# zhangxinsong-nlp/XFM

Measured on AMD Instinct MI355X. Metric: image-text pairs/sec fwd+bwd, XFM-base 224px/30tok, higher is better.
Workload: dtype bf16; 1 GPU; Pretrain.py full multimodal step (ITC+ITM+MLM+MIM), XFM-base, synthetic 224px images + 30-token captions, random init; units_per_gpu=64, global_batch=64, dropout=True, ordered_reductions=True, grad_allreduce=False, parallelism=dp1, image_res=224

## Files before the change

### xfm_amd/csrc/gemm.hip

```cpp
#include "gemm_common.h"
#include <limits.h>
#include "gemm_nt_small.hip"
#include "gemm_nt_256.hip"
#include "nt320_gemm.hip"
#include "gemm_tn_small.hip"
#include "gemm_tn_256.hip"
#include "gemm_cast.hip"

static int nt_k_slices(int M, int N, int K) {
  const long t = (long)cdiv(M, 64) * cdiv(N, 128);
  if (K < 8192 || t >= 192) return 1;
  int sp = (int)(512 / t);
  if (sp > K / 1024) sp = K / 1024;
  return sp < 1 ? 1 : sp;
}

static int nt_plan(int M, int N, int K, long lda, long ldb, int epi, int tile_hint, int* rows_a_out, int* k_splits_out) {
  *rows_a_out = 0;
  *k_splits_out = 1;
  if (tile_hint == 6) {
    static const int nt320_env = xfm_env_int("XFM_GEMM_NT320", 1);
    if (nt320_env && nt320_eligible(M, lda, N, ldb, K)) return 6;
    tile_hint = 0;
  }
  int cfg = tile_hint;
  if (cfg <= 0) {
    static const int split_env = xfm_env_int("XFM_GEMM_TAIL_SPLIT", 35);
    const long tn256 = cdiv(N, 256), t256 = (long)cdiv(M, 256) * tn256;
    if (split_env && tile_hint == 0 && M >= 2048 && t256 > 256 && t256 % 256 != 0 && (t256 % 256) * 100 < split_env * 256) {
      const int rows_a = (int)((t256 / 256) * 256 / tn256) * 256;
      if (rows_a > 0 && rows_a < M) {
        if (!nt256_eligible(rows_a, lda, N, ldb)) return 1;
        *rows_a_out = rows_a;
        return 5;
      }
    }
    if (M >= 2048 && (t256 >= 180 || (t256 >= 120 && M >= 8192))) cfg = nt256_eligible(M, lda, N, ldb) ? 5 : 1;
    else if (M >= 2048 && t256 >= 120) cfg = 1;
    else if ((long)cdiv(M, 256) * cdiv(N, 128) >= 768) cfg = 4;
    else if ((long)cdiv(M, 128) * cdiv(N, 128) >= 800) cfg = 1;
    else if ((long)cdiv(M, 64) * cdiv(N, 128) >= 512) cfg = 2;
    else if (K >= 1536 && epi != EPI_F32_ACC && (long)cdiv(M, 64) * cdiv(N, 128) < 300) {
      cfg = 8;
    }
    else if ((long)cdiv(M, 64) * cdiv(N, 128) >= 128 || K >= 1536) {
      cfg = 7;
      if (epi == EPI_F32_ACC) *k_splits_out = nt_k_slices(M, N, K);
    }
    else cfg = 3;
  }
  return cfg;
}

int xfm_gemm_nt_plan_impl(int M, int N, int K, int epi, int tile_hint, int* cfg, int* rows_a) {
  XFM_REQUIRE(M > 0 && N > 0 && K > 0 && cfg != nullptr && rows_a != nullptr, "gemm_nt_plan: bad arguments");
  int ks = 1;
  *cfg = nt_plan(M, N, K, K, K, epi, tile_hint, rows_a, &ks);
  return XFM_OK;
}

static GemmNT gemm_nt_args(const void* A, long lda, const void* B, long ldb, void* C, long ldc, const float* bias, int M, int N, int K) {
  static const int gm_env = xfm_env_int("XFM_GEMM_GROUP_M", 0);
  GemmNT g{};
  g.A = (const bf16*)A; g.lda = lda;
  g.B = (const bf16*)B; g.ldb = ldb;
  g.C = C; g.ldc = ldc;
  g.bias = bias;
  g.M = M; g.N = N; g.K = K;
  g.group_m = gm_env > 0 ? gm_env : 8;
  g.k_splits = 1;
  return g;
}

int xfm_gemm_nt_impl(const void* A, long lda, const void* B, long ldb, void* C, long ldc, const float* bias,
                     void* aux, long ldaux, int M, int N, int K, int epi, int tile_hint, hipStream_t st) {
  XFM_REQUIRE(M > 0 && N > 0 && K > 0, "gemm_nt: empty problem M=%d N=%d K=%d", M, N, K);
  XFM_REQUIRE(K % 64 == 0, "gemm_nt: K=%d must be a multiple of 64", K);
  XFM_REQUIRE(lda % 8 == 0 && ldb % 8 == 0, "gemm_nt: lda=%ld ldb=%ld must be multiples of 8", lda, ldb);
  XFM_REQUIRE(((uintptr_t)A % 16) == 0 && ((uintptr_t)B % 16) == 0 && ((uintptr_t)C % 16) == 0,
              "gemm_nt: operands must be 16-byte aligned");
  XFM_REQUIRE((epi != EPI_GELU && epi != EPI_DGELU) || aux != nullptr, "gemm_nt: epilogue %d needs aux", epi);
  GemmNT g = gemm_nt_args(A, lda, B, ldb, C, ldc, bias, M, N, K);
  g.aux = (bf16*)aux; g.ldaux = ldaux;
  int rows_a = 0, k_splits = 1;
  const int cfg = nt_plan(M, N, K, lda, ldb, epi, tile_hint, &rows_a, &k_splits);
  if (rows_a > 0) {
    int rc = xfm_gemm_nt_impl(A, lda, B, ldb, C, ldc, bias, aux, ldaux, rows_a, N, K, epi, 5, st);
    if (rc != XFM_OK) return rc;
    const long esz = (epi == EPI_F32 || epi == EPI_F32_ACC) ? 4 : 2;
    return xfm_gemm_nt_impl((const bf16*)A + (long)rows_a * lda, lda, B, ldb, (char*)C + (long)rows_a * ldc * esz, ldc, bias,
                            aux ? (void*)((bf16*)aux + (long)rows_a * ldaux) : nullptr, ldaux, M - rows_a, N, K, epi, -1, st);
  }
  g.k_splits = k_splits;
  switch (cfg) {
    case 1: return launch_nt<128, 128, 2>(g, epi, st);
    case 2: return launch_nt<64, 128, 2>(g, epi, st);
    case 7: return launch_nt<64, 128, 3>(g, epi, st);
    case 8: return launch_nt<64, 64, 4>(g, epi, st);
    case 4: return launch_nt_ring(g, epi, st);
    case 5: return launch_nt_256(g, epi, st);
    case 6: return launch_nt_320(g, epi, st);
    default: return launch_nt<64, 64, 2>(g, epi, st);
  }
}

// ... 343 lines not shown
```

### xfm_amd/csrc/nt320_gemm.hip

```cpp

constexpr int NT320_UNIT = 64 * 128;
constexpr int NT320_LEAD = 11;
constexpr int NT320_LDS = 18 * NT320_UNIT;

template <int V>
struct Nt320Phase { static constexpr int v = V; };

__device__ __forceinline__ void nt320_wait(int n) {
  if (n >= 10) wait_vm<10>();
  else if (n == 9) wait_vm<9>();
  else if (n == 8) wait_vm<8>();
  else if (n == 7) wait_vm<7>();
  else if (n == 6) wait_vm<6>();
  else if (n == 5) wait_vm<5>();
  else if (n == 4) wait_vm<4>();
  else if (n == 3) wait_vm<3>();
  else if (n == 2) wait_vm<2>();
  else if (n == 1) wait_vm<1>();
  else wait_vm<0>();
}

template <int EPI>
__global__ __launch_bounds__(512) void gemm_nt_320_kernel(GemmNT g) {
  constexpr int BM = 320, BN = 256, MT = 10, NT = 4, UNIT = NT320_UNIT, LEAD = NT320_LEAD;
  extern __shared__ __attribute__((aligned(16))) char smem[];
  const int tid = threadIdx.x, lane = tid & 63, w = __builtin_amdgcn_readfirstlane(tid >> 6);
  const int wr = w >> 2, wc = w & 3;
  const int lr = lane & 15, lg = lane >> 4;
  const int tiles_n = (g.N + BN - 1) / BN, tiles_m = (g.M + BM - 1) / BM;
  const int nk = g.K / 64;
  int tm, tn;
  grouped_tile(xcd_remap(blockIdx.x, tiles_m * tiles_n), tiles_m, tiles_n, g.group_m, tm, tn);
  const int m0 = tm * BM, n0 = tn * BN;

  unsigned soff[9];
  {
    const int ur = w * 8 + (lane >> 3);
#pragma unroll
    for (int u = 0; u < 5; ++u) {
      const int r = (ur & 31) + 32 * u + (ur >> 5) * 160;
      int gr = m0 + r; gr = gr < g.M ? gr : g.M - 1;
      soff[u == 0 ? 0 : 4 + u] = (unsigned)gr * (unsigned)g.lda + (((lane & 7) ^ swz_x(r)) << 3);
    }
#pragma unroll
    for (int h = 0; h < 4; ++h) {
      const int r = h * 64 + ur;
      int gr = n0 + r; gr = gr < g.N ? gr : g.N - 1;
      soff[1 + h] = (unsigned)gr * (unsigned)g.ldb + (((lane & 7) ^ swz_w(r)) << 3);
    }
  }
  const unsigned lds0 = (unsigned)(uintptr_t)LDS_PTR(void, smem) + (unsigned)(w * 1024);
  auto issue = [&](int j, int kt) {
    if (kt >= nk) return;
    const bf16* src = ((j == 0 || j >= 5) ? g.A : g.B) + kt * 64;
    const unsigned lds_addr = lds0 + (unsigned)(((kt & 1) * 9 + j) * UNIT);
    asm volatile("s_mov_b32 m0, %1\n\ts_nop 0\n\tglobal_load_lds_dwordx4 %0, off" ::"v"(src + (size_t)soff[j]), "s"(lds_addr) : "memory", "m0");
  };

  f32x4 acc[MT][NT];
#pragma unroll
  for (int i = 0; i < MT; ++i)
#pragma unroll
    for (int j = 0; j < NT; ++j) acc[i][j] = f32x4{0.f, 0.f, 0.f, 0.f};

  const int xs = swz_x(lr);
  const int wu = 8 * (lr >> 2) + (lr & 3);
  const int ws = swz_w(wu);
  const int xbase0 = (wr * 32 + lr) * 128 + (((0 + lg) ^ xs) << 4), xbase1 = (wr * 32 + lr) * 128 + (((4 + lg) ^ xs) << 4);
  const int wbase0 = (1 + wc) * UNIT + wu * 128 + (((0 + lg) ^ ws) << 4), wbase1 = (1 + wc) * UNIT + wu * 128 + (((4 + lg) ^ ws) << 4);

  bf16x8 xa[2][2], wf[4][2];
  const int total = 9 * nk;

  auto phase = [&](auto P, int kt) {
    constexpr int p = decltype(P)::v;
    constexpr int cum = p == 4 ? 9 : 2 * (p + 1);
    constexpr int need = p == 4 ? 14 : 6 + p;
    if (p == 0) { issue(2, kt + 1); issue(3, kt + 1); }
    if (p == 1) { issue(4, kt + 1); issue(5, kt + 1); }
    if (p == 2) { issue(6, kt + 1); issue(7, kt + 1); }
    if (p == 3) { issue(8, kt + 1); issue(0, kt + 2); }
    if (p == 4) { issue(1, kt + 2); }
    const char* buf = smem + (kt & 1) * 9 * UNIT;
    const char* xslot = buf + (p == 0 ? 0 : 4 + p) * UNIT;
#pragma unroll
    for (int m = 0; m < 2; ++m) {
      xa[m][0] = *reinterpret_cast<const bf16x8*>(xslot + xbase0 + m * 2048);
      xa[m][1] = *reinterpret_cast<const bf16x8*>(xslot + xbase1 + m * 2048);
    }
    if (p == 0) {
#pragma unroll
      for (int n = 0; n < 4; ++n) {
        wf[n][0] = *reinterpret_cast<const bf16x8*>(buf + wbase0 + (n >> 1) * 4096 + (n & 1) * 512);
        wf[n][1] = *reinterpret_cast<const bf16x8*>(buf + wbase1 + (n >> 1) * 4096 + (n & 1) * 512);
      }
    }
    {
      const int rem = total - 9 * kt;
      if (rem >= LEAD + cum) wait_vm<LEAD + cum - need>();
      else nt320_wait(rem - need);
    }
    XFM_BAR();
    __builtin_amdgcn_s_setprio(1);
#pragma unroll
    for (int ks = 0; ks < 2; ++ks)
#pragma unroll
      for (int m = 0; m < 2; ++m)
#pragma unroll
        for (int n = 0; n < 4; ++n)
          acc[2 * p + m][n] = __builtin_amdgcn_mfma_f32_16x16x32_bf16(wf[n][ks], xa[m][ks], acc[2 * p + m][n], 0, 0, 0);
    __builtin_amdgcn_s_setprio(0);
    XFM_BAR();
  };

#pragma unroll
  for (int j = 0; j < 9; ++j) issue(j, 0);
  issue(0, 1);
  issue(1, 1);
  nt320_wait((LEAD < total ? LEAD : total) - 5);
  XFM_BAR();
  if (wr == 1) XFM_BAR();

  for (int kt = 0; kt < nk; ++kt) {
    phase(Nt320Phase<0>{}, kt);
    phase(Nt320Phase<1>{}, kt);
    phase(Nt320Phase<2>{}, kt);
    phase(Nt320Phase<3>{}, kt);
    phase(Nt320Phase<4>{}, kt);
  }
  if (wr == 0) XFM_BAR();
  if (EPI == EPI_DGELU) {
    gemm_epilogue<MT / 2, NT, EPI>(g, reinterpret_cast<f32x4(&)[MT / 2][NT]>(acc[0]), m0 + wr * 160, n0 + wc * 64, lr, lg);
    gemm_epilogue<MT / 2, NT, EPI>(g, reinterpret_cast<f32x4(&)[MT / 2][NT]>(acc[MT / 2]), m0 + wr * 160 + 80, n0 + wc * 64, lr, lg);
  } else {
    gemm_epilogue<MT, NT, EPI>(g, acc, m0 + wr * 160, n0 + wc * 64, lr, lg);
  }
}

static bool nt320_eligible(int M, long lda, int N, long ldb, int K) {
  static const int cus = xfm_cu_count() > 0 ? xfm_cu_count() : 256;
  return N % 256 == 0 && K % 64 == 0 && (long)cdiv(M, 320) * (N / 256) <= cus && nt256_eligible(M, lda, N, ldb);
}

static int launch_nt_320(const GemmNT& g, int epi, hipStream_t st) {
  if (!nt320_eligible(g.M, g.lda, g.N, g.ldb, g.K)) {
    xfm_set_error("gemm_nt: M=%d N=%d K=%d is no shape of the one-round 320x256 kernel", g.M, g.N, g.K);
    return XFM_E_ARG;
  }
  const int tiles = cdiv(g.M, 320) * (g.N / 256);
  const int rc = nt_with_epilogue(epi, [&](auto e) {
    constexpr int E = decltype(e)::value;
    lds_launch<gemm_nt_320_kernel<E>, NT320_LDS>(dim3(tiles), dim3(512), NT320_LDS, st, g);
  });
  return rc != XFM_OK ? rc : xfm_check_launch("gemm_nt_320");
}
```

### xfm_amd/side_stream.py

```python
import contextlib
import os

import torch

from . import functional as Fx
from . import marks as _marks


class _DeferredCall:
    persistent = False

    def __init__(self, fn, keep=()):
        self.fn, self.keep = fn, tuple(keep)

    def run(self):
        self.fn()


class _WgradStream:
    _streams = {}
    enabled = os.environ.get("XFM_WGRAD_STREAM", "1") != "0"
    priority = int(os.environ.get("XFM_WGRAD_PRIO", "0"))

    @classmethod
    def side_of(cls, device, launch):
        key = (device.index if device.index is not None else torch.cuda.current_device(), launch.cuda_stream)
        if key not in cls._streams:
            cls._streams[key] = torch.cuda.Stream(device=device, priority=cls.priority)
        return cls._streams[key]

    @classmethod
    def sides(cls, device_index):
        return {launch: side for (d, launch), side in list(cls._streams.items()) if d == device_index}

    def __init__(self, device, label=None):
        self.label = label
        if label is not None:
            _marks.mark(label + " begin")
        self.main = torch.cuda.current_stream(device)
        if label is not None:
            from .arena import grads_ready
            grads_ready(device)
        self.on = _WgradStream.enabled
        if self.on:
            self.side = _WgradStream.side_of(device, self.main)
            self.side.wait_stream(self.main)
        self.keep = []
        self.queue = []
        self.reduces = []

    def _hand_over(self, keep):
        if not self.on:
            return contextlib.nullcontext()
        ev = torch.cuda.Event()
        ev.record(self.main)
        self.side.wait_event(ev)
        self.keep.append(keep)
        return torch.cuda.stream(self.side)

    def defer_tn(self, dy, x, dw, dbias=None):
        self.queue.append((dy, x, dw, dbias))

    def defer_call(self, fn, keep=()):
        self.reduces.append(_DeferredCall(fn, keep))

    def defer_reduces(self, rq):
        self.reduces.append(rq)

    def flush(self):
        reduces = self.reduces
        self.reduces = [r for r in reduces if getattr(r, "persistent", False)]
        items, self.queue = self.queue, []
        if not (reduces or items):
            return
        by_m = {}
        for it in items:
            by_m.setdefault(it[0].shape[0], []).append(it)
        with self._hand_over((items, reduces)):
            for r in reduces:
                r.run()
            for group in by_m.values():
                Fx.gemm_tn_group(group)

    def gemm_tn(self, dy, x, dw, **kw):
        with self._hand_over((dy, x)):
            Fx.gemm_tn(dy, x, dw, **kw)

    def project(self, x, slot):
        if not self.on:
            return Fx.gemm_nt(x, slot.wb, slot.b), None
        with torch.cuda.stream(self.side):
            y = Fx.gemm_nt(x, slot.wb, slot.b)
            ev = torch.cuda.Event()
            ev.record(self.side)
        y.record_stream(self.main)
        return y, ev

    def take(self, pair):
        y, ev = pair
        if ev is not None:
            self.main.wait_event(ev)
        return y

    def run(self, fn, keep=()):
        with self._hand_over(tuple(keep)):
            return fn()

    def sync_side(self):
        if self.on:
            self.main.wait_stream(self.side)

    def join_at_end(self):
        self.flush()
        if self.on:
            main, side, keep = self.main, self.side, self.keep

            def rejoin():
                main.wait_stream(side)
                cur = torch.cuda.current_stream(main.device)
                if cur != main:
                    cur.wait_stream(side)
                keep.clear()
            torch.autograd.Variable._execution_engine.queue_callback(rejoin)
            self.keep = []
        else:
            self.keep.clear()

    def join(self):
        if self.label is not None:
            _marks.mark(self.label + " chain end")
        self.flush()
        if self.on:
            self.main.wait_stream(self.side)
        self.keep.clear()
        if self.label is not None:
            _marks.mark(self.label + " end")
```

### xfm_amd/vit_trunk.py

```python
import math
import os

import torch
import torch.nn as nn

from . import _lib
from . import functional as Fx
from .arena import LinearSlot, OwnsArena, ParamArena, arena_note_grad, arena_note_use, grad_of
from .ops import linear_slot
from .side_stream import _WgradStream

_FAST_DELTA = os.environ.get("XFM_ATTN_FAST_DELTA", "0") != "0"
_VIT_FUSED_BWD = os.environ.get("XFM_ATTN_VIT_BWD", "0") != "0"
_DEFER_WGRAD = os.environ.get("XFM_VIT_DEFER_WGRAD", "1") != "0"
_RELPOS_AHEAD = os.environ.get("XFM_VIT_RELPOS_AHEAD", "1") != "0"
_DEFER_LN = os.environ.get("XFM_VIT_DEFER_LN", "1") != "0"
_WGRAD_GROUP_BLOCKS = int(os.environ.get("XFM_VIT_WGRAD_GROUP", "0"))
_GRAD_CHUNK_BLOCKS = max(1, int(os.environ.get("XFM_VIT_GRAD_CHUNK", "4")))


class _Affine(nn.Module):

    def __init__(self, dim, eps):
        super().__init__()
        self.weight = nn.Parameter(torch.ones(dim))
        self.bias = nn.Parameter(torch.zeros(dim))
        self.eps = eps


class _Dense(nn.Module):

    def __init__(self, fin, fout, bias=True):
        super().__init__()
        self.weight = nn.Parameter(torch.empty(fout, fin))
        self.bias = nn.Parameter(torch.zeros(fout)) if bias else None
        nn.init.trunc_normal_(self.weight, std=0.02, a=-2.0, b=2.0)


class PatchEmbed(nn.Module):
    def __init__(self, img_size, patch_size, in_chans, embed_dim):
        super().__init__()
        self.img_size = (img_size, img_size)
        self.patch_size = (patch_size, patch_size)
        self.patch_shape = (img_size // patch_size, img_size // patch_size)
        self.num_patches = self.patch_shape[0] * self.patch_shape[1]
        self.proj = nn.Module()
        self.proj.weight = nn.Parameter(torch.empty(embed_dim, in_chans, patch_size, patch_size))
        self.proj.bias = nn.Parameter(torch.zeros(embed_dim))
        nn.init.kaiming_uniform_(self.proj.weight, a=math.sqrt(5))


class _FusedViT(OwnsArena, nn.Module):
    _rel_pos = False
    _pool_tail = False
    _draw_at_rate_zero = False
    _trunk_bwd_done = None
    _block_grad_hook = None
    _arena = None
    _dp_keep = None

    def _layer_scale(self, gamma, grad=False):
        if gamma is None:
            return self._ones, None
        return gamma, (grad_of(gamma) if grad else None)

    def linear_slots(self):
        self._slot_patch = LinearSlot("patch_embed", [self.patch_embed.proj.weight], [self.patch_embed.proj.bias])
        self._slot_patch.need_t = False
        self._slots = []
        out = [self._slot_patch]
        for i, blk in enumerate(self.blocks):
            s = {"qkv": LinearSlot(f"blocks.{i}.qkv", [blk.attn.qkv.weight], self._qkv_bias_parts(blk)),
                 "proj": LinearSlot(f"blocks.{i}.proj", [blk.attn.proj.weight], [blk.attn.proj.bias]),
                 "fc1": LinearSlot(f"blocks.{i}.fc1", [blk.mlp.fc1.weight], [blk.mlp.fc1.bias]),
                 "fc2": LinearSlot(f"blocks.{i}.fc2", [blk.mlp.fc2.weight], [blk.mlp.fc2.bias])}
            self._slots.append(s)
            out.extend(s.values())
        return out

    def attach(self, arena):
        self._arena = arena
        N = self.patch_embed.num_patches + 1
        self._bias_ld = (N + 15) // 16 * 16
        if self.blocks[0].gamma_1 is None:
            self._ones = torch.ones(self.embed_dim, dtype=torch.float32, device=arena.device)

    def finalize(self, device=None):
        device = device or self.cls_token.device
        self.attach(ParamArena(self, self.linear_slots(), device))
        self._own_arena = True
        return self

    def _ready(self):
        if self._arena is None or not self._arena.attached():
            if self._arena is not None and not self._own_arena:
                raise RuntimeError("parameters were moved after the arena was built; call finalize() again")
            self.finalize()

    def _patch_tokens(self, x):
        patches = Fx.patchify(x.float().contiguous(), self.patch_embed.patch_size[0])
        return linear_slot(patches, self._slot_patch, x_requires_grad=False, out_fp32=True).view(x.shape[0], -1, self.embed_dim)

    def _drop_path_scales(self, B, device):
        if not self.training or not (self._draw_at_rate_zero or any(b.drop_path_prob > 0 for b in self.blocks)):
            return None
        keep = self._dp_keep
        if keep is None or keep.device != device:
            keep = 1.0 - torch.tensor([[b.drop_path_prob] * 2 for b in self.blocks], device=device).view(-1, 2, 1)
            self._dp_keep = keep
        return (torch.rand(len(self.blocks), 2, B, device=device) < keep).float() / keep


def _bias_plan(N, need_grad, fused_bwd):
    if 64 < N <= 224:
        return True, True, bool(fused_bwd and need_grad)
    if N > 256 and need_grad:
        return False, True, True
    return True, False, False


def _block_bias(vit, blk, H, N, ld, need_grad):
    transposed, tiles_fwd, tiles_bwd = _bias_plan(N, need_grad, _VIT_FUSED_BWD)
    dense = Fx.relpos_gather(blk.attn.relative_position_bias_table, vit._index32, H, N, ld, transposed=transposed)
    dense, dense_t = dense if transposed else (dense, None)
    tiles = Fx.bias_tiles(dense, N, blk.attn.scale, fwd=True, bwd=tiles_bwd) if tiles_fwd else None
    return dense, dense_t, tiles


def _biases_ahead(vit, H, N, ld, need_grad, device):
    pre = _WgradStream(device)
    if not pre.on:
        return None
    with torch.cuda.stream(pre.side):
        ahead = [_block_bias(vit, blk, H, N, ld, need_grad) for blk in vit.blocks]
        ev_bias = torch.cuda.Event()
        ev_bias.record(pre.side)
    for triple in ahead:
        for t in triple[:2] + tuple(triple[2] or ()):
            if t is not None:
                t.record_stream(pre.main)
    pre.main.wait_event(ev_bias)
    return ahead


def _reduce_queue(wg, n_blocks, M, D, device):
    rq = Fx.ReduceQueue(device, 2 * n_blocks * ((_lib.load().xfm_layernorm_bwd_workspace(M, D, 2) + 255) // 256 * 256))
    wg.defer_reduces(rq)
    return rq


def _relpos_table_grad(vit, blk, ddense, H, N, ld):
    G = blk.attn.window_size[0]
    dtab = grad_of(blk.attn.relative_position_bias_table)
    if N > 256 and blk.attn.window_size[0] == blk.attn.window_size[1] and N == G * G + 1:
        return lambda: Fx.relpos_grid_grad(ddense, G, H, ld, dtab)
    return lambda: Fx.relpos_scatter_sorted(ddense, vit._relpos_order, vit._relpos_start, H, N, ld, dtab)


def _nt320_hint(M, D, device):
    if device.type != "cuda" or D % 256 != 0:
        return 0
    cus = torch.cuda.get_device_properties(device).multi_processor_count
    return 6 if -(-M // 320) * (D // 256) <= cus < -(-M // 256) * (D // 256) else 0


class _TrunkFn(torch.autograd.Function):

    @staticmethod
    def forward(ctx, x0, vit, dp):
        B, N, D = x0.shape
        M, H = B * N, vit.num_heads
        x = x0.reshape(M, D).contiguous()
        ld = vit._bias_ld
        blocks = vit.blocks
        need_grad = bool(ctx.needs_input_grad[0])
        saved = []
        n0 = blocks[0].norm1
        y, mean, rstd = Fx.ln_fwd(x, n0.weight, n0.bias, n0.eps)
        ctx.first = (x, mean, rstd)
        ctx.nxt = nxts = [blk.norm1 for blk in blocks[1:]] + [vit._final_norm]
        rel_pos = vit._rel_pos
        ctx.nt_hint = hint = _nt320_hint(M, D, x.device)
        ahead = _biases_ahead(vit, H, N, ld, need_grad, x.device) if rel_pos and x.is_cuda and _RELPOS_AHEAD else None
        for i, blk in enumerate(blocks):
            s = vit._slots[i]
            g1, _ = vit._layer_scale(blk.gamma_1)
            g2, _ = vit._layer_scale(blk.gamma_2)
            dense = dense_t = tiles = None
            if ahead is not None:
                dense, dense_t, tiles = ahead[i]
            elif rel_pos:
                dense, dense_t, tiles = _block_bias(vit, blk, H, N, ld, need_grad)
            qkv = Fx.gemm_nt(y, s["qkv"].wb, s["qkv"].b)
            if need_grad and (_FAST_DELTA or N > 256):
                ctxv, lse, ctxv_lo = Fx.attn_fwd(qkv[:, :D], qkv[:, D:2 * D], qkv[:, 2 * D:], B, H, N, N, blk.attn.scale, bias=dense, lo=True,
                                                 bias_tiles=tiles)
            else:
                (ctxv, lse), ctxv_lo = Fx.attn_fwd(qkv[:, :D], qkv[:, D:2 * D], qkv[:, 2 * D:], B, H, N, N, blk.attn.scale, bias=dense,
                                                   bias_tiles=tiles), None
            h1 = Fx.gemm_nt(ctxv, s["proj"].wb, s["proj"].b, tile_hint=hint)
            dp1 = None if dp is None else dp[i, 0]
            dp2 = None if dp is None else dp[i, 1]
            x1, y2, mean2, rstd2 = Fx.ln_ls_fwd(x, h1, g1, dp1, N, blk.norm2.weight, blk.norm2.bias, blk.norm2.eps)
            hact, u = Fx.gemm_nt(y2, s["fc1"].wb, s["fc1"].b, epi=Fx.EPI_GELU)
            h2 = Fx.gemm_nt(hact, s["fc2"].wb, s["fc2"].b, tile_hint=hint)
            nxt = nxts[i]
            x2, yn, meann, rstdn = Fx.ln_ls_fwd(x1, h2, g2, dp2, N, nxt.weight, nxt.bias, nxt.eps)
            saved.append((y, dense, qkv, ctxv, lse, h1, x1, mean2, rstd2, y2, u, hact, h2, x2, meann, rstdn, dp1, dp2, dense_t, ctxv_lo, tiles))
            x, y = x2, yn
        ctx.saved, ctx.vit, ctx.shape = saved, vit, (B, N, D)
        ctx.noted = need_grad
        if ctx.noted:
            arena_note_use(vit)
        ctx.pooled = bool(vit._pool_tail)
        if ctx.pooled:
            Fx.pool_rows_fwd_(y, B, N)
        return y.view(B, N, D)

    @staticmethod
    def backward(ctx, dy_out):
        vit, (B, N, D) = ctx.vit, ctx.shape
        M, H = B * N, vit.num_heads
        blocks = vit.blocks
        ld = vit._bias_ld
        hint = ctx.nt_hint
        prev = vit._trunk_bwd_done
        if prev is not None and dy_out.is_cuda:
            torch.cuda.current_stream(dy_out.device).wait_event(prev)
        dy = dy_out.reshape(M, D).contiguous()
        if ctx.pooled:
            dy = Fx.pool_rows_bwd(dy if dy.dtype == torch.bfloat16 else dy.to(torch.bfloat16), B, N)
        dstream = torch.zeros((M, D), dtype=torch.float32, device=dy.device)
        wg = _WgradStream(dy.device, "vit bwd")
        done = len(blocks)
        ddense_all = None
        queued = _DEFER_WGRAD and dy.is_cuda
        tn = wg.defer_tn if queued else wg.gemm_tn
        rq = _reduce_queue(wg, len(blocks), M, D, dy.device) if _DEFER_LN and dy.is_cuda else None
        g = grad_of
        for i in reversed(range(len(blocks))):
            blk, s, nxt = blocks[i], vit._slots[i], ctx.nxt[i]
            (y, dense, qkv, ctxv, lse, h1, x1, mean2, rstd2, y2, u, hact, h2, x2, meann, rstdn, dp1, dp2, dense_t, ctxv_lo, tiles) = ctx.saved[i]
            g1, dg1 = vit._layer_scale(blk.gamma_1, grad=True)
            g2, dg2 = vit._layer_scale(blk.gamma_2, grad=True)
            dh2 = Fx.ln_ls_bwd(dy, dstream, x2, meann, rstdn, nxt.weight, h2, g2, dp2, N, g(nxt.weight), g(nxt.bias),
                               s["fc2"].db, dg2, defer=rq)
            tn(dh2, hact, s["fc2"].dw)
            du = Fx.gemm_nt(dh2, s["fc2"].wt, epi=Fx.EPI_DGELU, aux=u, n=s["fc2"].K)
            tn(du, y2, s["fc1"].dw, dbias=s["fc1"].db)
            dy2 = Fx.gemm_nt(du, s["fc1"].wt, n=s["fc1"].K, tile_hint=hint)
            dh1 = Fx.ln_ls_bwd(dy2, dstream, x1, mean2, rstd2, blk.norm2.weight, h1, g1, dp1, N, g(blk.norm2.weight),
                               g(blk.norm2.bias), s["proj"].db, dg1, defer=rq)
            tn(dh1, ctxv, s["proj"].dw)
            dctx = Fx.gemm_nt(dh1, s["proj"].wt, n=s["proj"].K, tile_hint=hint)
            dqkv = torch.empty_like(qkv)
            ddense = None
            if dense is not None:
                if ddense_all is None:
                    ddense_all = torch.zeros((len(blocks),) + tuple(dense.shape), dtype=dense.dtype, device=dense.device)
                ddense = ddense_all[i]
            Fx.attn_bwd(dctx, qkv[:, :D], qkv[:, D:2 * D], qkv[:, 2 * D:], ctxv, lse, dqkv[:, :D], dqkv[:, D:2 * D],
                        dqkv[:, 2 * D:], B, H, N, N, blk.attn.scale, bias=dense, dbias=ddense, bias_t=dense_t, o_lo=ctxv_lo,
                        bias_tiles=tiles if (_VIT_FUSED_BWD or N > 256) else None)
            if dense is not None:
                fn = _relpos_table_grad(vit, blk, ddense, H, N, ld)
                if queued:
                    wg.defer_call(fn, keep=(ddense_all,))
                else:
                    fn()
            tn(dqkv, y, s["qkv"].dw, dbias=s["qkv"].db)
            dy = Fx.gemm_nt(dqkv, s["qkv"].wt, n=s["qkv"].K, tile_hint=hint)
            ctx.saved[i] = None
            if _WGRAD_GROUP_BLOCKS > 0 and i % _WGRAD_GROUP_BLOCKS == 0:
                wg.flush()
            if ctx.noted and i > 0 and i % _GRAD_CHUNK_BLOCKS == 0 and i + 1 < done:
                hook = vit._block_grad_hook
                if hook is not None and hook(vit, i + 1, done, wg):
                    done = i + 1
        x0, mean0, rstd0 = ctx.first
        n0 = blocks[0].norm1
        Fx.ln_bwd(dy, x0, mean0, rstd0, n0.weight, grad_of(n0.weight), grad_of(n0.bias), dx32=dstream, dx_accum=True)
        wg.join()
        if dstream.is_cuda:
            ev = torch.cuda.Event()
            ev.record(torch.cuda.current_stream(dstream.device))
            vit._trunk_bwd_done = ev
        if ctx.noted:
            arena_note_grad(vit)
        return dstream.view(B, N, D), None, None
```

### xfm_amd/xroberta.py

```python
import json
import os
from types import SimpleNamespace

import torch
import torch.nn as nn

from . import functional as Fx
from .arena import LinearSlot, OwnsArena, ParamArena, arena_note_grad, arena_note_use
from .vit_trunk import _Affine
from .decode import GenerationMixin, cached_forward
from .ops import grad_view, lm_head_ce, lm_head_logits
from .roberta_encoder import _EncoderFn, _LastLayerRowsFn, layer_saves_maps
from .roberta_layer import _next_seed, _seed_counter
from .roberta_native import _KV_AHEAD, _RL_DEFER_LN, _RL_DEFER_WGRAD, _EncoderFnNative
from .side_stream import _WgradStream

BF16, F32 = torch.bfloat16, torch.float32


class RobertaConfig:

    def __init__(self, **kw):
        d = dict(vocab_size=50265, hidden_size=768, num_hidden_layers=12, num_attention_heads=12, intermediate_size=3072,
                 hidden_act="gelu", hidden_dropout_prob=0.1, attention_probs_dropout_prob=0.1, max_position_embeddings=514,
                 type_vocab_size=1, initializer_range=0.02, layer_norm_eps=1e-5, pad_token_id=1, bos_token_id=0,
                 eos_token_id=2, fusion_layer=12, encoder_width=768, add_cross_attention=False)
        d.update(kw)
        self.__dict__.update(d)

    @classmethod
    def from_json_file(cls, path):
        with open(path) as f:
            return cls(**json.load(f))


class _Lin(nn.Module):
    def __init__(self, fin, fout, std):
        super().__init__()
        self.weight = nn.Parameter(torch.empty(fout, fin).normal_(0.0, std))
        self.bias = nn.Parameter(torch.zeros(fout))


class _Emb(nn.Module):
    def __init__(self, n, dim, std, padding_idx=None):
        super().__init__()
        self.weight = nn.Parameter(torch.empty(n, dim).normal_(0.0, std))
        self.padding_idx = padding_idx
        if padding_idx is not None:
            with torch.no_grad():
                self.weight[padding_idx].zero_()


class RobertaEmbeddings(nn.Module):
    def __init__(self, config):
        super().__init__()
        std = config.initializer_range
        self.word_embeddings = _Emb(config.vocab_size, config.hidden_size, std, config.pad_token_id)
        self.position_embeddings = _Emb(config.max_position_embeddings, config.hidden_size, std, config.pad_token_id)
        self.token_type_embeddings = _Emb(config.type_vocab_size, config.hidden_size, std)
        self.LayerNorm = _Affine(config.hidden_size, config.layer_norm_eps)
        self.register_buffer("position_ids", torch.arange(config.max_position_embeddings).expand((1, -1)))
        self.padding_idx = config.pad_token_id
        self.p_drop = config.hidden_dropout_prob


_F32_STREAM = os.environ.get("XFM_F32_STREAM", "1") != "0"
"""The residual stream of the text / fusion towers in fp32 (A/B knob; 0 = the bf16 stream of rounds 1-4).  The reference trains in mixed
precision: its Linears produce 16-bit outputs, but LayerNorm and the residual add run in fp32 (apex O1 / autocast lists), so every
post-LN sum `LayerNorm(dropout(h) + x)` (xroberta.py:300-304, 381-385) sees the UN-ROUNDED output of the previous LayerNorm and the
gradient of the residual branch travels in fp32 too.  With the stream on, every tower hand-over is a (bf16, fp32) pair: the bf16 tensor
feeds the GEMMs, its fp32 twin the next residual add; the two are separate autograd edges (bf16 gradient from the GEMM side, fp32 from
the LayerNorm side)."""

_NATIVE_LAYERS = os.environ.get("XFM_NATIVE_LAYERS", "1") != "0"


def twin_of(t):
    return getattr(t, "_xfm_f32", None) if _F32_STREAM else None


def with_twin(t, t32):
    if t32 is not None and _F32_STREAM:
        t._xfm_f32 = t32
    return t


def rowwise(fn, *tensors):
    out = fn(*tensors)
    twins = [twin_of(t) for t in tensors]
    if all(tw is not None for tw in twins):
        with_twin(out, fn(*twins))
    return out
# ... 79 lines not shown


class RobertaAttention(nn.Module):
    def __init__(self, config, is_cross_attention=False):
        super().__init__()
        self.self = RobertaSelfAttention(config, is_cross_attention)
        self.output = RobertaSelfOutput(config)


class RobertaIntermediate(nn.Module):
    def __init__(self, config):
        super().__init__()
        self.dense = _Lin(config.hidden_size, config.intermediate_size, config.initializer_range)


class RobertaLayer(nn.Module):
    def __init__(self, config, layer_num):
        super().__init__()
        self.attention = RobertaAttention(config)
        self.has_cross_attention = layer_num >= config.fusion_layer
        if self.has_cross_attention:
            self.layer_num = layer_num
            self.crossattention = RobertaAttention(config, is_cross_attention=True)
        self.intermediate = RobertaIntermediate(config)
        self.output = RobertaSelfOutput(config, fin=config.intermediate_size)

    def linear_slots(self, prefix):
        a = self.attention
        s = {"qkv": LinearSlot(prefix + "qkv", [a.self.query.weight, a.self.key.weight, a.self.value.weight],
                               [a.self.query.bias, a.self.key.bias, a.self.value.bias]),
             "o": LinearSlot(prefix + "o", [a.output.dense.weight], [a.output.dense.bias]),
             "i": LinearSlot(prefix + "i", [self.intermediate.dense.weight], [self.intermediate.dense.bias]),
             "out": LinearSlot(prefix + "out", [self.output.dense.weight], [self.output.dense.bias])}
        if self.has_cross_attention:
            c = self.crossattention
            s["q2"] = LinearSlot(prefix + "q2", [c.self.query.weight], [c.self.query.bias])
            s["kv2"] = LinearSlot(prefix + "kv2", [c.self.key.weight, c.self.value.weight], [c.self.key.bias, c.self.value.bias])
            s["o2"] = LinearSlot(prefix + "o2", [c.output.dense.weight], [c.output.dense.bias])
        self._s = s
        self._rlp = None
        return list(s.values())


class RobertaEncoder(nn.Module):
    def __init__(self, config):
        super().__init__()
        self.config = config
        self.layer = nn.ModuleList([RobertaLayer(config, i) for i in range(config.num_hidden_layers)])


class RobertaModel(nn.Module):
    embeddings_class = RobertaEmbeddings

    def __init__(self, config, add_pooling_layer=False):
        super().__init__()
        if add_pooling_layer:
            raise NotImplementedError("pooler is never built on the XFM path (xroberta.py:1167)")
        if config.hidden_size // config.num_attention_heads != 64:
            raise NotImplementedError("head_dim must be 64")
        self.config = config
        self.embeddings = self.embeddings_class(config)
        self.encoder = RobertaEncoder(config)
        self.pooler = None
        self._arena = None

    def linear_slots(self, prefix=""):
        out = []
        for i, layer in enumerate(self.encoder.layer):
            out.extend(layer.linear_slots(f"{prefix}layer.{i}."))
        return out

    def prefetch_cross_kv(self, encoder_hidden_states):
        enc = encoder_hidden_states
        if not (_KV_AHEAD and enc.is_cuda and enc.dtype == BF16 and enc.is_contiguous() and self._arena is not None):
            return
        enc = enc.reshape(-1, enc.shape[-1])
        layers = [layer for layer in self.encoder.layer if layer.has_cross_attention]
        if not layers:
            return
        arena = layers[0]._s["kv2"]._arena
        for layer in layers:
            layer._s["kv2"]._ensure()
        pre = _WgradStream(enc.device)
        self._kv_ahead = ((enc.data_ptr(), tuple(enc.shape), enc._version), {id(layer): pre.project(enc, layer._s["kv2"]) for layer in layers}, enc)

    def attach(self, arena):
        self._arena = arena

    def forward(self, input_ids=None, attention_mask=None, token_type_ids=None, position_ids=None, head_mask=None,
                inputs_embeds=None, encoder_embeds=None, encoder_hidden_states=None, encoder_attention_mask=None,
                past_key_values=None, use_cache=None, output_attentions=None, output_hidden_states=None, return_dict=None,
                is_decoder=False, mode='multi_modal', encoder_batch_index=None, grad_batch=None, pack=None, encoder_row_ranges=None,
                output_rows=None, cache_capacity=None):
        if any(v is not None for v in (token_type_ids, position_ids, head_mask, inputs_embeds)):
            raise NotImplementedError("token_type_ids/position_ids/head_mask/inputs_embeds are not used on the XFM path")
        if use_cache or past_key_values is not None:
            if any(v is not None for v in (encoder_embeds, grad_batch, pack, encoder_row_ranges, output_rows)):
                raise NotImplementedError("use_cache / past_key_values take input_ids only (no encoder_embeds, grad_batch, pack, row ranges)")
            return cached_forward(self, input_ids, attention_mask=attention_mask, past_key_values=past_key_values,
                                  encoder_hidden_states=encoder_hidden_states, encoder_attention_mask=encoder_attention_mask,
                                  is_decoder=is_decoder, mode=mode, encoder_batch_index=encoder_batch_index, cache_capacity=cache_capacity)
        if isinstance(encoder_hidden_states, (list, tuple)):
            raise NotImplementedError("per-layer encoder_hidden_states lists (xroberta.py:435-444) are outside the hot-path scope")
        if self._arena is None:
            raise RuntimeError("RobertaModel is not attached to a parameter arena; build it through XFMBase or call finalize()")
        cfg = self.config
        f32 = _F32_STREAM
        if pack is not None and is_decoder:
            raise NotImplementedError("packed rows are for the bidirectional towers")
        if encoder_embeds is None:
            if input_ids is None:
                raise ValueError("You have to specify either input_ids or inputs_embeds")
            B, T = input_ids.shape
            drop = Fx.drop_params(cfg.hidden_dropout_prob if self.training else 0.0, _next_seed())
            x, x32 = _EmbedFn.apply(self.embeddings.word_embeddings.weight, self.embeddings, input_ids, drop, self, pack, f32)
        else:
            if pack is not None:
                assert encoder_embeds.dim() == 2 and encoder_embeds.shape[0] == pack.cap, "packed encoder_embeds are [pack.cap, D] rows"
                B, T = pack.B, pack.T
            else:
                B, T = encoder_embeds.shape[:2]
            x32 = twin_of(encoder_embeds)
            if encoder_embeds.dtype == BF16:
                x = encoder_embeds
            else:
                x, x32 = encoder_embeds.to(BF16), (encoder_embeds if encoder_embeds.dtype == F32 and f32 else None)
        if pack is not None:
            assert (B, T) == (pack.B, pack.T)
            attention_mask = None
        dev = x.device
        key_keep = None if attention_mask is None else attention_mask.to(device=dev, dtype=torch.int32).contiguous()
        enc, enc_keep, Nenc = None, None, 0
        if encoder_hidden_states is not None:
            enc = encoder_hidden_states if encoder_hidden_states.dtype == BF16 else encoder_hidden_states.to(BF16)
            Nenc = enc.shape[1]
            enc = enc.reshape(-1, enc.shape[-1])
            if encoder_attention_mask is not None and not getattr(encoder_attention_mask, "_xfm_all_ones", False):
                enc_keep = encoder_attention_mask.to(device=dev, dtype=torch.int32).contiguous()
            if encoder_batch_index is not None:
                encoder_batch_index = encoder_batch_index.to(device=dev, dtype=torch.int32).contiguous()
                assert encoder_batch_index.numel() == B
        if mode == 'text':
            lo, hi = 0, cfg.fusion_layer
        elif mode == 'fusion':
            lo, hi = cfg.fusion_layer, cfg.num_hidden_layers
        elif mode == 'multi_modal':
            lo, hi = 0, cfg.num_hidden_layers
        else:
            raise ValueError(f"mode {mode} is not supported")
        y = x.reshape(B * T, -1) if pack is None else x
        y32 = None if x32 is None else (x32.reshape(B * T, -1) if pack is None else x32)
        if hi > lo:
            xq = None
            if encoder_row_ranges is not None and enc is not None:
                assert pack is not None and Nenc <= 256, "per-image row ranges need packed rows and <= 256 image tokens"
                xq = (encoder_row_ranges[0].to(device=dev, dtype=torch.int32).contiguous(),
                      encoder_row_ranges[1].to(device=dev, dtype=torch.int32).contiguous(), int(encoder_row_ranges[2]))
            native = _NATIVE_LAYERS and y.is_cuda and (enc is None or xq is not None or
                                                       (encoder_batch_index is not None and Fx.attn_grouped_ok(T, Nenc)))
            saving = enc is not None and any(layer_saves_maps(self.encoder.layer[li]) for li in range(lo, hi))
            fn = _EncoderFn if saving else (_EncoderFnNative if native else _EncoderFn)
            if output_rows is not None:
                assert pack is not None and xq is None and grad_batch is None and not is_decoder and key_keep is None
                assert enc is None or (encoder_batch_index is not None and Fx.attn_grouped_ok(int(output_rows[3]), Nenc))
                if saving and layer_saves_maps(self.encoder.layer[hi - 1]):
                    from .packing import rows_gather
                    y, y32 = fn.apply(y, y32, enc, self, key_keep, enc_keep, lo, hi, bool(is_decoder), B, T, Nenc, self.training,
# ... 141 lines not shown
```

Measured before the change: 1787 pairs/s.

## Add persistent multi-tile 320x256 NT GEMM overlapping next-tile prologue with epilogue

The 320x256 NT GEMM becomes a persistent kernel that loops over several tiles per workgroup. It issues the next tile's global-to-LDS prologue loads before running the current tile's epilogue stores, and relaxes vmcnt waits so those pending stores do not block the next tile. The tile-hint heuristic now counts rounds of workgroups against the CU count, so the kernel is also picked for multi-round shapes such as the ViT QKV projection and the cross-attention KV projection. The bias is staged through LDS. The cost is more complex counter accounting, and a mis-sized wait would be a correctness risk.

```diff
diff --git a/xfm_amd/csrc/gemm.hip b/xfm_amd/csrc/gemm.hip
--- a/xfm_amd/csrc/gemm.hip
+++ b/xfm_amd/csrc/gemm.hip
@@ -18,9 +18,9 @@
 static int nt_plan(int M, int N, int K, long lda, long ldb, int epi, int tile_hint, int* rows_a_out, int* k_splits_out) {
   *rows_a_out = 0;
   *k_splits_out = 1;
-  if (tile_hint == 6) {
+  if (tile_hint == 6 || tile_hint == 11) {
     static const int nt320_env = xfm_env_int("XFM_GEMM_NT320", 1);
-    if (nt320_env && nt320_eligible(M, lda, N, ldb, K)) return 6;
+    if (nt320_env && nt320_eligible(M, lda, N, ldb, K, tile_hint == 6)) return 6;
     tile_hint = 0;
   }
   int cfg = tile_hint;
diff --git a/xfm_amd/csrc/nt320_gemm.hip b/xfm_amd/csrc/nt320_gemm.hip
--- a/xfm_amd/csrc/nt320_gemm.hip
+++ b/xfm_amd/csrc/nt320_gemm.hip
@@ -6,49 +6,55 @@
 template <int V>
 struct Nt320Phase { static constexpr int v = V; };
 
+template <int NS = 0>
 __device__ __forceinline__ void nt320_wait(int n) {
-  if (n >= 10) wait_vm<10>();
-  else if (n == 9) wait_vm<9>();
-  else if (n == 8) wait_vm<8>();
-  else if (n == 7) wait_vm<7>();
-  else if (n == 6) wait_vm<6>();
-  else if (n == 5) wait_vm<5>();
-  else if (n == 4) wait_vm<4>();
-  else if (n == 3) wait_vm<3>();
-  else if (n == 2) wait_vm<2>();
-  else if (n == 1) wait_vm<1>();
-  else wait_vm<0>();
-}
-
-template <int EPI>
-__global__ __launch_bounds__(512) void gemm_nt_320_kernel(GemmNT g) {
+  if (n >= 10) wait_vm<10 + NS>();
+  else if (n == 9) wait_vm<9 + NS>();
+  else if (n == 8) wait_vm<8 + NS>();
+  else if (n == 7) wait_vm<7 + NS>();
+  else if (n == 6) wait_vm<6 + NS>();
+  else if (n == 5) wait_vm<5 + NS>();
+  else if (n == 4) wait_vm<4 + NS>();
+  else if (n == 3) wait_vm<3 + NS>();
+  else if (n == 2) wait_vm<2 + NS>();
+  else if (n == 1) wait_vm<1 + NS>();
+  else wait_vm<NS>();
+}
+
+template <int EPI, bool PERSIST>
+__device__ __forceinline__ void nt320_tiles(const GemmNT& g, const int tiles) {
   constexpr int BM = 320, BN = 256, MT = 10, NT = 4, UNIT = NT320_UNIT, LEAD = NT320_LEAD;
+  constexpr int NS = !PERSIST || EPI == EPI_F32_ACC ? 0 : EPI == EPI_BF16 ? 20 : 40;
+  static_assert(LEAD - 1 + NS <= 63, "vmcnt is a 6-bit counter");
   extern __shared__ __attribute__((aligned(16))) char smem[];
   const int tid = threadIdx.x, lane = tid & 63, w = __builtin_amdgcn_readfirstlane(tid >> 6);
   const int wr = w >> 2, wc = w & 3;
   const int lr = lane & 15, lg = lane >> 4;
   const int tiles_n = (g.N + BN - 1) / BN, tiles_m = (g.M + BM - 1) / BM;
   const int nk = g.K / 64;
-  int tm, tn;
-  grouped_tile(xcd_remap(blockIdx.x, tiles_m * tiles_n), tiles_m, tiles_n, g.group_m, tm, tn);
-  const int m0 = tm * BM, n0 = tn * BN;
 
   unsigned soff[9];
-  {
-    const int ur = w * 8 + (lane >> 3);
+  auto tile_origin = [&](int v, int& m0, int& n0) {
+    int tm, tn;
+    grouped_tile(xcd_remap(v, tiles), tiles_m, tiles_n, g.group_m, tm, tn);
+    m0 = tm * BM;
+    n0 = tn * BN;
+  };
+  auto tile_offsets = [&](int m0, int n0, int ln) {
+    const int ur = w * 8 + (ln >> 3);
 #pragma unroll
     for (int u = 0; u < 5; ++u) {
       const int r = (ur & 31) + 32 * u + (ur >> 5) * 160;
       int gr = m0 + r; gr = gr < g.M ? gr : g.M - 1;
-      soff[u == 0 ? 0 : 4 + u] = (unsigned)gr * (unsigned)g.lda + (((lane & 7) ^ swz_x(r)) << 3);
+      soff[u == 0 ? 0 : 4 + u] = (unsigned)gr * (unsigned)g.lda + (((ln & 7) ^ swz_x(r)) << 3);
     }
 #pragma unroll
     for (int h = 0; h < 4; ++h) {
       const int r = h * 64 + ur;
       int gr = n0 + r; gr = gr < g.N ? gr : g.N - 1;
-      soff[1 + h] = (unsigned)gr * (unsigned)g.ldb + (((lane & 7) ^ swz_w(r)) << 3);
-    }
-  }
+      soff[1 + h] = (unsigned)gr * (unsigned)g.ldb + (((ln & 7) ^ swz_w(r)) << 3);
+    }
+  };
   const unsigned lds0 = (unsigned)(uintptr_t)LDS_PTR(void, smem) + (unsigned)(w * 1024);
   auto issue = [&](int j, int kt) {
     if (kt >= nk) return;
@@ -56,12 +62,14 @@
     const unsigned lds_addr = lds0 + (unsigned)(((kt & 1) * 9 + j) * UNIT);
     asm volatile("s_mov_b32 m0, %1\n\ts_nop 0\n\tglobal_load_lds_dwordx4 %0, off" ::"v"(src + (size_t)soff[j]), "s"(lds_addr) : "memory", "m0");
   };
+  auto prologue = [&]() {
+#pragma unroll
+    for (int j = 0; j < 9; ++j) issue(j, 0);
+    issue(0, 1);
+    issue(1, 1);
+  };
 
   f32x4 acc[MT][NT];
-#pragma unroll
-  for (int i = 0; i < MT; ++i)
-#pragma unroll
-    for (int j = 0; j < NT; ++j) acc[i][j] = f32x4{0.f, 0.f, 0.f, 0.f};
 
   const int xs = swz_x(lr);
   const int wu = 8 * (lr >> 2) + (lr & 3);
@@ -72,7 +80,7 @@
   bf16x8 xa[2][2], wf[4][2];
   const int total = 9 * nk;
 
-  auto phase = [&](auto P, int kt) {
+  auto phase = [&](auto P, int kt, bool behind) {
     constexpr int p = decltype(P)::v;
     constexpr int cum = p == 4 ? 9 : 2 * (p + 1);
     constexpr int need = p == 4 ? 14 : 6 + p;
@@ -97,8 +105,13 @@
     }
     {
       const int rem = total - 9 * kt;
-      if (rem >= LEAD + cum) wait_vm<LEAD + cum - need>();
-      else nt320_wait(rem - need);
+      if (NS > 0 && p < 4 && behind) {
+        if (rem >= LEAD + cum) wait_vm<LEAD + cum - need + NS>();
+        else nt320_wait<NS>(rem - need);
+      } else {
+        if (rem >= LEAD + cum) wait_vm<LEAD + cum - need>();
+        else nt320_wait(rem - need);
+      }
     }
     XFM_BAR();
     __builtin_amdgcn_s_setprio(1);
@@ -113,44 +126,101 @@
     XFM_BAR();
   };
 
-#pragma unroll
-  for (int j = 0; j < 9; ++j) issue(j, 0);
-  issue(0, 1);
-  issue(1, 1);
-  nt320_wait((LEAD < total ? LEAD : total) - 5);
-  XFM_BAR();
-  if (wr == 1) XFM_BAR();
-
-  for (int kt = 0; kt < nk; ++kt) {
-    phase(Nt320Phase<0>{}, kt);
-    phase(Nt320Phase<1>{}, kt);
-    phase(Nt320Phase<2>{}, kt);
-    phase(Nt320Phase<3>{}, kt);
-    phase(Nt320Phase<4>{}, kt);
+  int v = blockIdx.x, m0, n0;
+  tile_origin(v, m0, n0);
+  tile_offsets(m0, n0, lane);
+  prologue();
+  bool stores_behind = false;
+
+  while (true) {
+#pragma unroll
+    for (int i = 0; i < MT; ++i)
+#pragma unroll
+      for (int j = 0; j < NT; ++j) acc[i][j] = f32x4{0.f, 0.f, 0.f, 0.f};
+    if (NS > 0 && stores_behind) nt320_wait<NS>((LEAD < total ? LEAD : total) - 5);
+    else nt320_wait((LEAD < total ? LEAD : total) - 5);
+    XFM_BAR();
+    if (wr == 1) XFM_BAR();
+
+    for (int kt = 0; kt < nk; ++kt) {
+      const bool behind = NS > 0 && stores_behind && kt == 0;
+      phase(Nt320Phase<0>{}, kt, behind);
+      phase(Nt320Phase<1>{}, kt, behind);
+      phase(Nt320Phase<2>{}, kt, behind);
+      phase(Nt320Phase<3>{}, kt, behind);
+      phase(Nt320Phase<4>{}, kt, behind);
+    }
+    if (wr == 0) XFM_BAR();
+    const int cm0 = m0, cn0 = n0;
+    const float* lds_bias = nullptr;
+    bool more = false;
+    int elr = lr, elg = lg;
+    if (PERSIST) {
+      int ln = lane;
+      asm volatile("" : "+v"(ln));
+      elr = ln & 15;
+      elg = ln >> 4;
+      float* lb = reinterpret_cast<float*>(smem + 17 * UNIT + w * 256);
+      if (g.bias != nullptr) {
+        int col = cn0 + wc * 64 + ln;
+        col = col < g.N ? col : g.N - 1;
+        const unsigned lds_addr = (unsigned)(uintptr_t)LDS_PTR(void, lb);
+        asm volatile("s_mov_b32 m0, %1\n\ts_nop 0\n\tglobal_load_lds_dword %0, off" ::"v"(g.bias + col), "s"(lds_addr) : "memory", "m0");
+      } else {
+        lb[ln] = 0.f;
+      }
+      v += gridDim.x;
+      more = v < tiles;
+      if (more) {
+        tile_origin(v, m0, n0);
+        tile_offsets(m0, n0, ln);
+        prologue();
+      }
+      if (!more) wait_vm<0>();
+      else if (nk == 1) wait_vm<9>();
+      else wait_vm<LEAD>();
+      if (g.bias == nullptr) asm volatile("s_waitcnt lgkmcnt(0)" ::: "memory");
+      lds_bias = lb;
+    }
+    if (EPI == EPI_DGELU) {
+      gemm_epilogue<MT / 2, NT, EPI>(g, reinterpret_cast<f32x4(&)[MT / 2][NT]>(acc[0]), cm0 + wr * 160, cn0 + wc * 64, elr, elg, lds_bias);
+      gemm_epilogue<MT / 2, NT, EPI>(g, reinterpret_cast<f32x4(&)[MT / 2][NT]>(acc[MT / 2]), cm0 + wr * 160 + 80, cn0 + wc * 64, elr, elg, lds_bias);
+    } else {
+      gemm_epilogue<MT, NT, EPI>(g, acc, cm0 + wr * 160, cn0 + wc * 64, elr, elg, lds_bias);
+    }
+    if (!more) break;
+    XFM_FENCE();
+    stores_behind = cm0 + BM <= g.M && cn0 + BN <= g.N && (g.ldc % 8) == 0 && ((EPI != EPI_GELU && EPI != EPI_DGELU) || (g.ldaux % 8) == 0);
   }
-  if (wr == 0) XFM_BAR();
-  if (EPI == EPI_DGELU) {
-    gemm_epilogue<MT / 2, NT, EPI>(g, reinterpret_cast<f32x4(&)[MT / 2][NT]>(acc[0]), m0 + wr * 160, n0 + wc * 64, lr, lg);
-    gemm_epilogue<MT / 2, NT, EPI>(g, reinterpret_cast<f32x4(&)[MT / 2][NT]>(acc[MT / 2]), m0 + wr * 160 + 80, n0 + wc * 64, lr, lg);
-  } else {
-    gemm_epilogue<MT, NT, EPI>(g, acc, m0 + wr * 160, n0 + wc * 64, lr, lg);
-  }
-}
-
-static bool nt320_eligible(int M, long lda, int N, long ldb, int K) {
+}
+
+template <int EPI>
+__global__ __launch_bounds__(512) void gemm_nt_320_kernel(GemmNT g) {
+  nt320_tiles<EPI, false>(g, ((g.M + 319) / 320) * ((g.N + 255) / 256));
+}
+template <int EPI>
+__global__ __launch_bounds__(512) void gemm_nt_320_persist_kernel(GemmNT g, int tiles) {
+  nt320_tiles<EPI, true>(g, tiles);
+}
+
+static bool nt320_eligible(int M, long lda, int N, long ldb, int K, bool one_round) {
   static const int cus = xfm_cu_count() > 0 ? xfm_cu_count() : 256;
-  return N % 256 == 0 && K % 64 == 0 && (long)cdiv(M, 320) * (N / 256) <= cus && nt256_eligible(M, lda, N, ldb);
+  return N % 256 == 0 && K % 64 == 0 && (!one_round || (long)cdiv(M, 320) * (N / 256) <= cus) && nt256_eligible(M, lda, N, ldb);
 }
 
 static int launch_nt_320(const GemmNT& g, int epi, hipStream_t st) {
-  if (!nt320_eligible(g.M, g.lda, g.N, g.ldb, g.K)) {
-    xfm_set_error("gemm_nt: M=%d N=%d K=%d is no shape of the one-round 320x256 kernel", g.M, g.N, g.K);
+  if (!nt320_eligible(g.M, g.lda, g.N, g.ldb, g.K, false)) {
+    xfm_set_error("gemm_nt: M=%d N=%d K=%d is no shape of the 320x256 kernel", g.M, g.N, g.K);
     return XFM_E_ARG;
   }
   const int tiles = cdiv(g.M, 320) * (g.N / 256);
+  static const int persist_env = xfm_env_int("XFM_GEMM_PERSIST", 1);
+  static const int cus = xfm_cu_count();
+  const bool persist = persist_env && cus >= 8 && tiles > cus;
   const int rc = nt_with_epilogue(epi, [&](auto e) {
     constexpr int E = decltype(e)::value;
-    lds_launch<gemm_nt_320_kernel<E>, NT320_LDS>(dim3(tiles), dim3(512), NT320_LDS, st, g);
+    if (persist) lds_launch<gemm_nt_320_persist_kernel<E>, NT320_LDS>(dim3(cus & ~7), dim3(512), NT320_LDS, st, g, tiles);
+    else lds_launch<gemm_nt_320_kernel<E>, NT320_LDS>(dim3(tiles), dim3(512), NT320_LDS, st, g);
   });
   return rc != XFM_OK ? rc : xfm_check_launch("gemm_nt_320");
 }
diff --git a/xfm_amd/side_stream.py b/xfm_amd/side_stream.py
--- a/xfm_amd/side_stream.py
+++ b/xfm_amd/side_stream.py
@@ -86,11 +86,11 @@
         with self._hand_over((dy, x)):
             Fx.gemm_tn(dy, x, dw, **kw)
 
-    def project(self, x, slot):
+    def project(self, x, slot, tile_hint=0):
         if not self.on:
-            return Fx.gemm_nt(x, slot.wb, slot.b), None
+            return Fx.gemm_nt(x, slot.wb, slot.b, tile_hint=tile_hint), None
         with torch.cuda.stream(self.side):
-            y = Fx.gemm_nt(x, slot.wb, slot.b)
+            y = Fx.gemm_nt(x, slot.wb, slot.b, tile_hint=tile_hint)
             ev = torch.cuda.Event()
             ev.record(self.side)
         y.record_stream(self.main)
diff --git a/xfm_amd/vit_trunk.py b/xfm_amd/vit_trunk.py
--- a/xfm_amd/vit_trunk.py
+++ b/xfm_amd/vit_trunk.py
@@ -1,3 +1,4 @@
+import functools
 import math
 import os
 
@@ -157,11 +158,13 @@
     return lambda: Fx.relpos_scatter_sorted(ddense, vit._relpos_order, vit._relpos_start, H, N, ld, dtab)
 
 
-def _nt320_hint(M, D, device):
-    if device.type != "cuda" or D % 256 != 0:
+@functools.lru_cache(maxsize=None)
+def _nt320_hint(M, N, device):
+    if device.type != "cuda" or N % 256 != 0:
         return 0
     cus = torch.cuda.get_device_properties(device).multi_processor_count
-    return 6 if -(-M // 320) * (D // 256) <= cus < -(-M // 256) * (D // 256) else 0
+    rounds = lambda rows: -(-(-(-M // rows) * (N // 256)) // cus)
+    return 0 if rounds(320) >= rounds(256) else 6 if rounds(320) == 1 else 11
 
 
 class _TrunkFn(torch.autograd.Function):
@@ -180,7 +183,8 @@
         ctx.first = (x, mean, rstd)
         ctx.nxt = nxts = [blk.norm1 for blk in blocks[1:]] + [vit._final_norm]
         rel_pos = vit._rel_pos
-        ctx.nt_hint = hint = _nt320_hint(M, D, x.device)
+        hint = _nt320_hint(M, D, x.device)
+        hint_qkv = _nt320_hint(M, vit._slots[0]["qkv"].N, x.device)
         ahead = _biases_ahead(vit, H, N, ld, need_grad, x.device) if rel_pos and x.is_cuda and _RELPOS_AHEAD else None
         for i, blk in enumerate(blocks):
             s = vit._slots[i]
@@ -191,7 +195,7 @@
                 dense, dense_t, tiles = ahead[i]
             elif rel_pos:
                 dense, dense_t, tiles = _block_bias(vit, blk, H, N, ld, need_grad)
-            qkv = Fx.gemm_nt(y, s["qkv"].wb, s["qkv"].b)
+            qkv = Fx.gemm_nt(y, s["qkv"].wb, s["qkv"].b, tile_hint=hint_qkv)
             if need_grad and (_FAST_DELTA or N > 256):
                 ctxv, lse, ctxv_lo = Fx.attn_fwd(qkv[:, :D], qkv[:, D:2 * D], qkv[:, 2 * D:], B, H, N, N, blk.attn.scale, bias=dense, lo=True,
                                                  bias_tiles=tiles)
@@ -223,7 +227,7 @@
         M, H = B * N, vit.num_heads
         blocks = vit.blocks
         ld = vit._bias_ld
-        hint = ctx.nt_hint
+        hint = _nt320_hint(M, D, dy_out.device)
         prev = vit._trunk_bwd_done
         if prev is not None and dy_out.is_cuda:
             torch.cuda.current_stream(dy_out.device).wait_event(prev)
diff --git a/xfm_amd/xroberta.py b/xfm_amd/xroberta.py
--- a/xfm_amd/xroberta.py
+++ b/xfm_amd/xroberta.py
@@ -7,7 +7,7 @@
 
 from . import functional as Fx
 from .arena import LinearSlot, OwnsArena, ParamArena, arena_note_grad, arena_note_use
-from .vit_trunk import _Affine
+from .vit_trunk import _Affine, _nt320_hint
 from .decode import GenerationMixin, cached_forward
 from .ops import grad_view, lm_head_ce, lm_head_logits
 from .roberta_encoder import _EncoderFn, _LastLayerRowsFn, layer_saves_maps
@@ -253,7 +253,9 @@
         for layer in layers:
             layer._s["kv2"]._ensure()
         pre = _WgradStream(enc.device)
-        self._kv_ahead = ((enc.data_ptr(), tuple(enc.shape), enc._version), {id(layer): pre.project(enc, layer._s["kv2"]) for layer in layers}, enc)
+        hint = _nt320_hint(enc.shape[0], layers[0]._s["kv2"].N, enc.device)
+        self._kv_ahead = ((enc.data_ptr(), tuple(enc.shape), enc._version), {id(layer): pre.project(enc, layer._s["kv2"], hint) for layer in layers},
+                          enc)
 
     def attach(self, arena):
         self._arena = arena
```

Result: no change. 1782 pairs/s (median of 5 runs) (-0.3%).
